# Orbiter-Finance/Plonky2-lib

Hardware: AMD Instinct MI355X
Metric: proofs/sec for secp256k1 ECDSA-verify circuit; Goldilocks NTT GB/s vs HBM peak (higher is better)
Workload: dtype u64 (Goldilocks, 64-bit modular integer)

## Files before the change

### include/glp.h

```cpp
#ifndef GLP_H
#define GLP_H
#include <stddef.h>
#include <stdint.h>

#ifdef __cplusplus
extern "C" {
#endif

#if defined(__GNUC__)
#define GLP_API __attribute__((visibility("default")))
#else
#define GLP_API
#endif

#define GLP_OK 0
#define GLP_ERR_ARG (-1)
#define GLP_ERR_HIP (-2)
#define GLP_ERR_UNSUPPORTED (-3)
#define GLP_ERR_NOGPU (-4)
#define GLP_ERR_PROVE (-5)

#define GLP_HASH_POSEIDON 0
#define GLP_HASH_KECCAK25 1

typedef struct glp_ctx glp_ctx;
typedef struct glp_batch glp_batch;

GLP_API const char *glp_last_error(void);
GLP_API const char *glp_version(void);
GLP_API int glp_device_count(void);

GLP_API int glp_ctx_create(int device_id, glp_ctx **out);
GLP_API void glp_ctx_destroy(glp_ctx *ctx);
GLP_API int glp_ctx_synchronize(glp_ctx *ctx);
GLP_API void *glp_ctx_stream(glp_ctx *ctx);
GLP_API int glp_ctx_set_salt_seed(glp_ctx *ctx, const uint64_t seed[4]);

GLP_API int glp_dev_alloc(glp_ctx *ctx, size_t bytes, void **dev_out);
GLP_API int glp_dev_free(glp_ctx *ctx, void *dev);
GLP_API int glp_dev_upload(glp_ctx *ctx, void *dev_dst, const void *host_src, size_t bytes);
GLP_API int glp_dev_download(glp_ctx *ctx, void *host_dst, const void *dev_src, size_t bytes);

GLP_API int glp_ctx_set_profiling(glp_ctx *ctx, int on);
GLP_API int glp_ctx_stage_reset(glp_ctx *ctx);
GLP_API int glp_ctx_stage_count(glp_ctx *ctx);
GLP_API int glp_ctx_stage_get(glp_ctx *ctx, int index, const char **name, float *ms, double *algorithmic_bytes);

GLP_API int glp_poseidon_permute(glp_ctx *ctx, uint64_t *states, size_t count);
GLP_API int glp_fft(glp_ctx *ctx, uint64_t *cols, uint32_t ncols, uint32_t log_n);
GLP_API int glp_ifft(glp_ctx *ctx, uint64_t *cols, uint32_t ncols, uint32_t log_n);
GLP_API int glp_lde(glp_ctx *ctx, const uint64_t *coeffs, uint32_t ncols, uint32_t log_n, uint32_t rate_bits,
            uint64_t shift, uint64_t *out);

GLP_API int glp_fill_random_device(glp_ctx *ctx, uint64_t *dev_out, size_t count, uint64_t seed);

GLP_API int glp_batch_from_values(glp_ctx *ctx, const uint64_t *values, uint32_t ncols, uint32_t log_n,
                          uint32_t rate_bits, uint32_t cap_height, glp_batch **out);
GLP_API int glp_batch_from_values_device(glp_ctx *ctx, const uint64_t *dev_values, uint32_t ncols, uint32_t log_n,
                                 uint32_t rate_bits, uint32_t cap_height, glp_batch **out);
GLP_API int glp_batch_from_coeffs(glp_ctx *ctx, const uint64_t *coeffs, uint32_t ncols, uint32_t log_n,
                          uint32_t rate_bits, uint32_t cap_height, glp_batch **out);
GLP_API int glp_batch_from_coeffs_device(glp_ctx *ctx, const uint64_t *dev_coeffs, uint32_t ncols, uint32_t log_n,
                                 uint32_t rate_bits, uint32_t cap_height, glp_batch **out);
GLP_API int glp_batch_from_values_h(glp_ctx *ctx, const uint64_t *values, uint32_t ncols, uint32_t log_n, uint32_t rate_bits,
                                    uint32_t cap_height, uint32_t hasher, glp_batch **out);
#define GLP_SALT_SIZE 4
#define GLP_SALT_TAG_WIRES 0
#define GLP_SALT_TAG_ZS 1
#define GLP_SALT_TAG_QUOTIENT 2
#define GLP_SALT_TAG_BATCH 3
GLP_API int glp_batch_from_values_salted(glp_ctx *ctx, const uint64_t *values, uint32_t ncols, uint32_t log_n, uint32_t rate_bits,
                                         uint32_t cap_height, uint32_t hasher, const uint64_t seed[4], glp_batch **out);
GLP_API uint32_t glp_batch_leaf_len(const glp_batch *b);
GLP_API int glp_batch_from_coeffs_h(glp_ctx *ctx, const uint64_t *coeffs, uint32_t ncols, uint32_t log_n, uint32_t rate_bits,
                                    uint32_t cap_height, uint32_t hasher, glp_batch **out);
GLP_API int glp_keccak256(glp_ctx *ctx, const uint8_t *msgs, size_t count, size_t len, uint8_t *digests_out);
GLP_API void glp_batch_free(glp_batch *b);
GLP_API int glp_batch_info(const glp_batch *b, uint32_t *ncols, uint32_t *log_n, uint32_t *rate_bits, uint32_t *cap_height);
GLP_API int glp_batch_cap(const glp_batch *b, uint64_t *cap_out);
GLP_API int glp_batch_coeffs(const glp_batch *b, uint32_t col_begin, uint32_t ncols, uint64_t *out);
GLP_API int glp_batch_leaf(const glp_batch *b, uint64_t leaf_index, uint64_t *out );
// ... 184 lines not shown
```

### plonky2-lib_amd/binding.py

```python
import ctypes as C
import os
import re
import subprocess
import weakref

import numpy as np

P = 0xFFFFFFFF00000001
_HERE = os.path.dirname(os.path.abspath(__file__))
_ROOT = os.path.dirname(_HERE)
_SO = os.path.join(_HERE, "libglprover.so")
_lib = None


class GlpError(RuntimeError):
    def __init__(self, code, msg):
        super().__init__("glp error %d: %s" % (code, msg))
        self.code = code


class _Gate(C.Structure):
    _fields_ = [(f, C.c_uint32) for f in ("type", "selector_index", "group_start", "group_end", "row",
                                          "num_constraints", "p0", "p1")]

# ... 32 lines not shown
        args.append("-B")
    subprocess.check_call(args, stdout=subprocess.DEVNULL)
    return _SO


def exported_symbols():
    hdr = open(os.path.join(_ROOT, "include", "glp.h")).read()
    return re.findall(r"GLP_API [^;(]*?(glp_\w+)\(", hdr)


def load_library():
    global _lib
    if _lib is not None:
        return _lib
    if not os.path.exists(_SO):
        raise GlpError(-4, "libglprover.so is not built (run __graft_entry__.build()); there is no CPU fallback")
    L = C.CDLL(_SO)
    vp, u32, u64, sz = C.c_void_p, C.c_uint32, C.c_uint64, C.c_size_t
    L.glp_last_error.restype = C.c_char_p
    L.glp_version.restype = C.c_char_p
    L.glp_ctx_stream.restype = vp
    L.glp_ctx_stream.argtypes = [vp]
    L.glp_batch_num_digests.restype = sz
    L.glp_batch_num_digests.argtypes = [vp]
    sigs = {
        "glp_ctx_create": [C.c_int, C.POINTER(vp)],
        "glp_ctx_destroy": [vp],
        "glp_ctx_synchronize": [vp],
        "glp_ctx_set_profiling": [vp, C.c_int],
        "glp_ctx_stage_reset": [vp],
        "glp_ctx_stage_count": [vp],
        "glp_ctx_stage_get": [vp, C.c_int, C.POINTER(C.c_char_p), C.POINTER(C.c_float), C.POINTER(C.c_double)],
        "glp_poseidon_permute": [vp, vp, sz],
        "glp_fill_random_device": [vp, vp, sz, u64],
        "glp_fft": [vp, vp, u32, u32],
        "glp_ifft": [vp, vp, u32, u32],
        "glp_lde": [vp, vp, u32, u32, u32, u64, vp],
        "glp_batch_from_values": [vp, vp, u32, u32, u32, u32, C.POINTER(vp)],
        "glp_batch_from_values_device": [vp, vp, u32, u32, u32, u32, C.POINTER(vp)],
        "glp_batch_from_coeffs": [vp, vp, u32, u32, u32, u32, C.POINTER(vp)],
        "glp_batch_from_coeffs_device": [vp, vp, u32, u32, u32, u32, C.POINTER(vp)],
        "glp_batch_from_values_h": [vp, vp, u32, u32, u32, u32, u32, C.POINTER(vp)],
        "glp_batch_from_coeffs_h": [vp, vp, u32, u32, u32, u32, u32, C.POINTER(vp)],
        "glp_keccak256": [vp, vp, sz, sz, vp],
        "glp_batch_free": [vp],
        "glp_batch_info": [vp, C.POINTER(u32), C.POINTER(u32), C.POINTER(u32), C.POINTER(u32)],
        "glp_batch_cap": [vp, vp],
        "glp_batch_coeffs": [vp, u32, u32, vp],
        "glp_batch_leaf": [vp, u64, vp],
        "glp_batch_merkle_proof": [vp, u64, vp],
        "glp_batch_digests": [vp, vp],
        "glp_batch_from_values_salted": [vp, vp, u32, u32, u32, u32, u32, vp, C.POINTER(vp)],
        "glp_ctx_set_salt_seed": [vp, vp],
    }
    L.glp_batch_leaf_len.restype = u32
    L.glp_batch_leaf_len.argtypes = [vp]
    for name in ("glp_batch_num_proofs", "glp_fri_num_proofs"):
        getattr(L, name).restype = u32
        getattr(L, name).argtypes = [vp]
    L.glp_proof_words.restype = sz
    L.glp_proof_words.argtypes = [vp]
    L.glp_proof_bytes_len.restype = sz
    L.glp_proof_bytes_len.argtypes = [vp]
    sigs.update({
        "glp_circuit_create": [vp, C.POINTER(_CircuitDesc), C.POINTER(vp)],
        "glp_circuit_create_ex": [vp, C.POINTER(_CircuitDesc), u32, C.POINTER(vp)],
# ... 943 lines not shown
```

### plonky2-lib_amd/csrc/fri_kernels.inc

```
struct ZTArgs { u64 *zt; ext2 zp2[24]; u32 lg; const u64 *zeta_b; size_t zeta_stride; };
template <bool BATCH>
__global__ __launch_bounds__(256) void k_zeta_table(ZTArgs a) {
    const size_t n = (size_t)1 << a.lg;
    const size_t p = (size_t)blockIdx.x * 256 + threadIdx.x;
    if (p >= n) return;
    const u32 k = bitrev32((u32)p, a.lg);
    ext2 acc = e_from(1);
    if constexpr (BATCH) {
        const u64 *z = a.zeta_b + (size_t)blockIdx.y * a.zeta_stride;
        ext2 sq = e_make(z[0], z[1]);
        for (u32 b = 0; b < a.lg; b++) { if ((k >> b) & 1) acc = e_mul(acc, sq); sq = e_sqr(sq); }
        a.zt += (size_t)blockIdx.y * 2 * n;
    } else {
        for (u32 b = 0; b < a.lg; b++) if ((k >> b) & 1) acc = e_mul(acc, a.zp2[b]);
    }
    a.zt[2 * p] = acc.a; a.zt[2 * p + 1] = acc.b;
}
constexpr int OPEN_BLOCKS = 32;
inline u32 open_blocks(size_t n) { return (u32)std::max<size_t>(1, std::min<size_t>(OPEN_BLOCKS, n / 256)); }
__global__ __launch_bounds__(256) void k_open_dot(const u64 *coeffs, const u64 *zt, u64 *partial, u32 lg, size_t coeffs_bstride,
                                                  size_t zt_bstride, size_t partial_bstride) {
    __shared__ u64 sa[256], sb[256];
    coeffs += (size_t)blockIdx.z * coeffs_bstride; zt += (size_t)blockIdx.z * zt_bstride; partial += (size_t)blockIdx.z * partial_bstride;
    const size_t n = (size_t)1 << lg;
// ... 316 lines not shown
    }
    sa[t] = red.a; sb[t] = red.b;
    __syncthreads();
    for (int s = 128; s > 0; s >>= 1) { if ((int)t < s) { sa[t] = add(sa[t], sa[t + s]); sb[t] = add(sb[t], sb[t + s]); } __syncthreads(); }
    if (t == 0) {
        u64 *pp = a.pp + pk * FCM_PP_WORDS;
        const ext2 shift = e_pow(alpha, len);
        pp[2 * b] = sa[0]; pp[2 * b + 1] = sb[0];
        pp[2 * (NP + b)] = a.z[2 * (pk * npoints + b)]; pp[2 * (NP + b) + 1] = a.z[2 * (pk * npoints + b) + 1];
        pp[2 * (2 * NP + b)] = shift.a; pp[2 * (2 * NP + b) + 1] = shift.b;
    }
}
__global__ __launch_bounds__(256) void k_scale_bitrev_pow(u64 *data, u64 base, u32 lg) {
    const size_t n = (size_t)1 << lg;
    const size_t p = (size_t)blockIdx.x * 256 + threadIdx.x;
    if (p >= n) return;
    const u64 f = dpow(base, bitrev32((u32)p, lg));
    data[(size_t)blockIdx.y * n + p] = mul(data[(size_t)blockIdx.y * n + p], f);
}

__global__ __launch_bounds__(256, 4) void k_fri_leaf_hash(const u64 *vals, u64 *digests, u32 lgL, u32 rb, u32 ab, size_t vals_bstride,
                                                       size_t dig_bstride) {
    vals += (size_t)blockIdx.y * vals_bstride; digests += (size_t)blockIdx.y * dig_bstride;
    const size_t L = (size_t)1 << lgL, ncur = L >> rb, nleaves = L >> ab;
    const size_t Mp = (size_t)blockIdx.x * 256 + threadIdx.x;
    if (Mp >= nleaves) return;
    const size_t m = bitrev32((u32)Mp, lgL - ab);
    const u32 arity = 1u << ab;
    u64 s[12];
#pragma unroll
    for (int i = 0; i < 12; i++) s[i] = 0;
    const u64 *re = vals, *im = vals + L;
    u32 fill = 0;
    for (u32 t = 0; t < arity; t++) {
        const size_t i = (size_t)bitrev32(t, ab) * nleaves + Mp;
        const size_t pos = (i & (((size_t)1 << rb) - 1)) * ncur + (i >> rb);
        s[fill++] = re[pos];
        s[fill++] = im[pos];
        if (fill == 8) { if (2 * arity > 4) pos::permute(s); fill = 0; }
    }
    if (fill && 2 * arity > 4) pos::permute(s);
    ulonglong2 d0, d1;
    d0.x = s[0]; d0.y = s[1]; d1.x = s[2]; d1.y = s[3];
    reinterpret_cast<ulonglong2 *>(digests + 4 * m)[0] = d0;
    reinterpret_cast<ulonglong2 *>(digests + 4 * m)[1] = d1;
}
__global__ __launch_bounds__(256) void k_fri_leaf_hash_coop(const u64 *vals, u64 *digests, u32 lgL, u32 rb, u32 ab, size_t vals_bstride,
                                                            size_t dig_bstride) {
    vals += (size_t)blockIdx.y * vals_bstride; digests += (size_t)blockIdx.y * dig_bstride;
    const size_t L = (size_t)1 << lgL, ncur = L >> rb, nleaves = L >> ab;
    const int tid = threadIdx.x, l = tid & 15, lane = tid & 63, group_base = lane & ~15;
    const size_t Mp0 = (size_t)blockIdx.x * 16 + (tid >> 4);
    const bool live = Mp0 < nleaves;
    const size_t Mp = live ? Mp0 : 0;
    const size_t m = bitrev32((u32)Mp, lgL - ab);
    const u32 len = 2u << ab;
    u64 x = 0;
    for (u32 c = 0; c < len; c += 8) {
        if (l < 8 && c + l < len) {
            const u32 e = c + l, t = e >> 1;
            const size_t i = (size_t)bitrev32(t, ab) * nleaves + Mp;
            const size_t pos = (i & (((size_t)1 << rb) - 1)) * ncur + (i >> rb);
            x = vals[(e & 1 ? L : 0) + pos];
        }
        if (len > 4) x = pos::permute_coop(x, l, group_base);
    }
    if (live && l < 4) digests[4 * m + l] = x;
}
__global__ __launch_bounds__(256) void k_fri_leaf_hash_quad(const u64 *vals, u64 *digests, u32 lgL, u32 rb, u32 ab, size_t vals_bstride,
                                                            size_t dig_bstride) {
    vals += (size_t)blockIdx.y * vals_bstride; digests += (size_t)blockIdx.y * dig_bstride;
    const size_t L = (size_t)1 << lgL, ncur = L >> rb, nleaves = L >> ab;
    const int tid = threadIdx.x, q = tid & 3;
    const size_t Mp0 = (size_t)blockIdx.x * 64 + (tid >> 2);
// ... 185 lines not shown
```

### plonky2-lib_amd/csrc/merkle.hip

```cpp
#include "merkle.h"
#include "keccak.h"
#include "poseidon.h"

namespace glp {
using namespace glf;

constexpr size_t MERKLE_COOP_MAX_PARENTS = 8192;

size_t merkle_num_digests(size_t nleaves, int cap_height) {
    size_t t = 0, w = nleaves, cap = (size_t)1 << cap_height;
    for (;;) { t += w; if (w <= cap) break; w >>= 1; }
    return t;
}
size_t merkle_cap_offset(size_t nleaves, int cap_height) {
    return merkle_num_digests(nleaves, cap_height) - ((size_t)1 << cap_height);
}

__device__ __forceinline__ void store_digest(u64 *dst, const u64 s[12]) {
    ulonglong2 a, b;
    a.x = s[0]; a.y = s[1]; b.x = s[2]; b.y = s[3];
    reinterpret_cast<ulonglong2 *>(dst)[0] = a;
    reinterpret_cast<ulonglong2 *>(dst)[1] = b;
}

__global__ __launch_bounds__(256, 4) void k_leaf_hash_lde(const u64 *__restrict__ lde, u64 *__restrict__ digests,
                                                       u32 ncols, int lg, int rate_bits, size_t lde_stride, size_t dig_stride) {
    lde += (size_t)blockIdx.y * lde_stride; digests += (size_t)blockIdx.y * dig_stride;
    const size_t N = (size_t)1 << (lg + rate_bits);
    const size_t pos = (size_t)blockIdx.x * 256 + threadIdx.x;
    if (pos >= N) return;
    const u32 r = (u32)(pos >> lg), q = (u32)(pos & (((size_t)1 << lg) - 1));
    const size_t leaf = ((size_t)bitrev32(r, rate_bits) << lg) | bitrev32(q, lg);
    u64 s[12];
#pragma unroll
    for (int i = 0; i < 12; i++) s[i] = 0;
    const u64 *p = lde + pos;
    if (ncols <= 4) {
        for (u32 c = 0; c < ncols; c++) s[c] = p[(size_t)c * N];
    } else {
        u64 nx[8];
#pragma unroll
        for (int i = 0; i < 8; i++) nx[i] = i < (int)ncols ? p[(size_t)i * N] : 0;
        for (u32 c = 0; c < ncols; c += 8) {
#pragma unroll
            for (int i = 0; i < 8; i++)
                if (c + i < ncols) s[i] = nx[i];
            if (c + 8 < ncols) {
#pragma unroll
                for (int i = 0; i < 8; i++)
                    if (c + 8 + i < ncols) nx[i] = p[(size_t)(c + 8 + i) * N];
            }
            pos::permute(s);
        }
    }
    store_digest(digests + 4 * leaf, s);
}

__global__ __launch_bounds__(256) void k_leaf_hash_lde_coop(const u64 *__restrict__ lde, u64 *__restrict__ digests,
                                                            u32 ncols, int lg, int rate_bits, size_t lde_stride, size_t dig_stride) {
    lde += (size_t)blockIdx.y * lde_stride; digests += (size_t)blockIdx.y * dig_stride;
    const size_t N = (size_t)1 << (lg + rate_bits);
    const int tid = threadIdx.x, l = tid & 15, lane = tid & 63, group_base = lane & ~15;
    const size_t pos = (size_t)blockIdx.x * 16 + (tid >> 4);
    const bool live = pos < N;
    const size_t p = live ? pos : 0;
    const u32 r = (u32)(p >> lg), q = (u32)(p & (((size_t)1 << lg) - 1));
    const size_t leaf = ((size_t)bitrev32(r, rate_bits) << lg) | bitrev32(q, lg);
    u64 x = 0;
    if (ncols <= 4) {
        if (live && l < 4) digests[4 * leaf + l] = (u32)l < ncols ? lde[(size_t)l * N + p] : 0;
        return;
    }
    for (u32 c = 0; c < ncols; c += 8) {
        if (l < 8 && c + l < ncols) x = lde[(size_t)(c + l) * N + p];
        x = pos::permute_coop(x, l, group_base);
    }
    if (live && l < 4) digests[4 * leaf + l] = x;
}

__global__ __launch_bounds__(256) void k_leaf_hash_lde_quad(const u64 *__restrict__ lde, u64 *__restrict__ digests,
                                                            u32 ncols, int lg, int rate_bits, size_t lde_stride, size_t dig_stride) {
    lde += (size_t)blockIdx.y * lde_stride; digests += (size_t)blockIdx.y * dig_stride;
    const size_t N = (size_t)1 << (lg + rate_bits);
    const int tid = threadIdx.x, q = tid & 3;
    const size_t pos = (size_t)blockIdx.x * 64 + (tid >> 2);
// ... 5 lines not shown
        if (live) digests[4 * leaf + q] = (u32)q < ncols ? lde[(size_t)q * N + p] : 0;
        return;
    }
    u64 x[3] = {0, 0, 0};
    for (u32 c = 0; c < ncols; c += 8) {
#pragma unroll
        for (int s = 0; s < 3; s++) {
            const u32 e = 3 * q + s;
            if (e < 8 && c + e < ncols) x[s] = lde[(size_t)(c + e) * N + p];
        }
        pos::permute_quad(x, q);
    }
    if (live) {
        if (q == 0) { digests[4 * leaf] = x[0]; digests[4 * leaf + 1] = x[1]; digests[4 * leaf + 2] = x[2]; }
        if (q == 1) digests[4 * leaf + 3] = x[0];
    }
}

__global__ __launch_bounds__(256, 4) void k_leaf_hash_rows(const u64 *__restrict__ rows, u64 *__restrict__ digests,
                                                        size_t nleaves, u32 leaf_len) {
    const size_t j = (size_t)blockIdx.x * 256 + threadIdx.x;
    if (j >= nleaves) return;
    u64 s[12];
#pragma unroll
    for (int i = 0; i < 12; i++) s[i] = 0;
    const u64 *p = rows + j * leaf_len;
    if (leaf_len <= 4) {
        for (u32 c = 0; c < leaf_len; c++) s[c] = p[c];
    } else {
        u32 c = 0;
        for (; c + 8 <= leaf_len; c += 8) {
#pragma unroll
            for (int i = 0; i < 8; i++) s[i] = p[c + i];
            pos::permute(s);
        }
        if (c < leaf_len) {
#pragma unroll
            for (int i = 0; i < 8; i++)
                if (c + i < leaf_len) s[i] = p[c + i];
            pos::permute(s);
        }
    }
    store_digest(digests + 4 * j, s);
}

__global__ __launch_bounds__(256) void k_merkle_level(const u64 *__restrict__ in, u64 *__restrict__ out, size_t m, size_t dig_stride) {
    in += (size_t)blockIdx.y * dig_stride; out += (size_t)blockIdx.y * dig_stride;
    const size_t i = (size_t)blockIdx.x * 256 + threadIdx.x;
    if (i >= m) return;
    const ulonglong2 *src = reinterpret_cast<const ulonglong2 *>(in + 8 * i);
    ulonglong2 a = src[0], b = src[1], c2 = src[2], d = src[3];
    u64 s[12] = {a.x, a.y, b.x, b.y, c2.x, c2.y, d.x, d.y, 0, 0, 0, 0};
    pos::permute(s);
    store_digest(out + 4 * i, s);
}

__global__ __launch_bounds__(256) void k_merkle_level_coop(const u64 *__restrict__ in, u64 *__restrict__ out, size_t m, size_t dig_stride) {
    in += (size_t)blockIdx.y * dig_stride; out += (size_t)blockIdx.y * dig_stride;
    const int tid = threadIdx.x, l = tid & 15, lane = tid & 63, group_base = lane & ~15;
    const size_t i = (size_t)blockIdx.x * 16 + (tid >> 4);
    const bool live = i < m;
    u64 x = (live && l < 8) ? in[8 * i + l] : 0;
    x = pos::permute_coop(x, l, group_base);
    if (live && l < 4) out[4 * i + l] = x;
}

__global__ __launch_bounds__(256) void k_merkle_level_quad(const u64 *__restrict__ in, u64 *__restrict__ out, size_t m, size_t dig_stride) {
    in += (size_t)blockIdx.y * dig_stride; out += (size_t)blockIdx.y * dig_stride;
    const int tid = threadIdx.x, q = tid & 3;
    const size_t i0 = (size_t)blockIdx.x * 64 + (tid >> 2);
    const bool live = i0 < m;
    const size_t i = live ? i0 : 0;
    u64 x[3];
#pragma unroll
    for (int s = 0; s < 3; s++) x[s] = 3 * q + s < 8 ? in[8 * i + 3 * q + s] : 0;
    pos::permute_quad(x, q);
    if (live) {
        if (q == 0) { out[4 * i] = x[0]; out[4 * i + 1] = x[1]; out[4 * i + 2] = x[2]; }
        if (q == 1) out[4 * i + 3] = x[0];
    }
}

__global__ void k_permute_states(u64 *states, size_t count) {
    const size_t i = (size_t)blockIdx.x * blockDim.x + threadIdx.x;
    if (i >= count) return;
    u64 s[12];
#pragma unroll
    for (int k = 0; k < 12; k++) s[k] = states[12 * i + k];
    pos::permute(s);
#pragma unroll
    for (int k = 0; k < 12; k++) states[12 * i + k] = s[k];
}

__global__ __launch_bounds__(256) void k_leaf_hash_lde_keccak(const u64 *__restrict__ lde, u64 *__restrict__ digests, u32 ncols, int lg,
                                                              int rate_bits, size_t lde_stride, size_t dig_stride) {
    lde += (size_t)blockIdx.y * lde_stride; digests += (size_t)blockIdx.y * dig_stride;
    const size_t N = (size_t)1 << (lg + rate_bits);
    const size_t pos = (size_t)blockIdx.x * 256 + threadIdx.x;
    if (pos >= N) return;
    const u32 r = (u32)(pos >> lg), q = (u32)(pos & (((size_t)1 << lg) - 1));
    const size_t leaf = ((size_t)bitrev32(r, rate_bits) << lg) | bitrev32(q, lg);
    const u64 *p = lde + pos;
    u64 d[4] = {0, 0, 0, 0};
    if (ncols <= 3) {
        for (u32 c = 0; c < ncols; c++) d[c] = p[(size_t)c * N];
    } else {
        kec::Sponge s;
        kec::sponge_init(s);
        u32 c = 0;
        for (; c + kec::RATE_LANES <= ncols; c += kec::RATE_LANES) {
#pragma unroll
            for (int i = 0; i < kec::RATE_LANES; i++) s.a[i] ^= p[(size_t)(c + i) * N];
            kec::f1600(s.a);
        }
#pragma unroll
        for (int i = 0; i < kec::RATE_LANES; i++) if (c + i < ncols) s.a[i] ^= p[(size_t)(c + i) * N];
        s.fill = (int)(ncols - c);
        kec::sponge_finish(s);
        kec::sponge_digest25(s, d);
    }
    store_digest(digests + 4 * leaf, d);
}
__global__ __launch_bounds__(256) void k_merkle_level_keccak(const u64 *__restrict__ in, u64 *__restrict__ out, size_t m, size_t dig_stride) {
    in += (size_t)blockIdx.y * dig_stride; out += (size_t)blockIdx.y * dig_stride;
    const size_t i = (size_t)blockIdx.x * 256 + threadIdx.x;
    if (i >= m) return;
    const ulonglong2 *src = reinterpret_cast<const ulonglong2 *>(in + 8 * i);
    const ulonglong2 a = src[0], b = src[1], c2 = src[2], e = src[3];
    const u64 l[4] = {a.x, a.y, b.x, b.y}, r[4] = {c2.x, c2.y, e.x, e.y};
    u64 d[4];
    kec::two_to_one(l, r, d);
    store_digest(out + 4 * i, d);
}

static int build_levels(glp_ctx *c, u64 *dev_digests, size_t nleaves, int cap_height, u32 K = 1, size_t dig_stride = 0, int hasher = 0) {
    size_t w = nleaves, cap = (size_t)1 << cap_height;
    u64 *lvl = dev_digests;
    while (w > cap) {
        u64 *nxt = lvl + 4 * w;
        size_t m = w >> 1;
        if (hasher == GLP_HASH_KECCAK25)
            hipLaunchKernelGGL(k_merkle_level_keccak, dim3((unsigned)((m + 255) / 256), K), dim3(256), 0, c->stream, lvl, nxt, m, dig_stride);
        else if (m * K <= MERKLE_COOP_MAX_PARENTS)
            hipLaunchKernelGGL(k_merkle_level_coop, dim3((unsigned)((m + 15) / 16), K), dim3(256), 0, c->stream, lvl, nxt, m, dig_stride);
        else if (m * K <= c->merkle_quad_max)
            hipLaunchKernelGGL(k_merkle_level_quad, dim3((unsigned)((m + 63) / 64), K), dim3(256), 0, c->stream, lvl, nxt, m, dig_stride);
        else
            hipLaunchKernelGGL(k_merkle_level, dim3((unsigned)((m + 255) / 256), K), dim3(256), 0, c->stream, lvl, nxt, m, dig_stride);
        GLP_HIP(hipGetLastError());
        lvl = nxt; w = m;
    }
    return GLP_OK;
}

int merkle_levels(glp_ctx *c, u64 *dev_digests, size_t nleaves, int cap_height, u32 K, size_t dig_stride, int hasher) {
    return build_levels(c, dev_digests, nleaves, cap_height, K, dig_stride, hasher);
}

int merkle_from_lde(glp_ctx *c, const u64 *dev_lde, u32 ncols, int lg, int rate_bits, int cap_height, u64 *dev_digests, u32 K,
                    size_t lde_stride, size_t dig_stride, int hasher) {
    const size_t N = (size_t)1 << (lg + rate_bits);
    if (cap_height < 0 || ((size_t)1 << cap_height) > N)
        return set_error(GLP_ERR_ARG, "cap_height=%d should be at most log2(leaves)=%d", cap_height, lg + rate_bits);
    GLP_REQUIRE(K >= 1 && K <= 65535, "batch of %u trees outside 1..65535", K);
    {
        StageScope st(c, "merkle_leaves", (double)N * K * (8.0 * ncols + 32.0));
        if (hasher == GLP_HASH_KECCAK25)
            hipLaunchKernelGGL(k_leaf_hash_lde_keccak, dim3((unsigned)((N + 255) / 256), K), dim3(256), 0, c->stream, dev_lde, dev_digests,
                               ncols, lg, rate_bits, lde_stride, dig_stride);
        else if (N * K <= c->merkle_coop_max)
            hipLaunchKernelGGL(k_leaf_hash_lde_coop, dim3((unsigned)((N + 15) / 16), K), dim3(256), 0, c->stream, dev_lde, dev_digests,
                               ncols, lg, rate_bits, lde_stride, dig_stride);
        else if (N * K <= c->merkle_quad_max)
// ... 72 lines not shown
__global__ __launch_bounds__(256) void k_salt_lde(u64 *__restrict__ lde, u32 ncols, int lg, int rate_bits, size_t lde_stride,
                                                  u64 seed0, u64 seed1, u64 seed2, u64 seed3, u32 tag) {
    lde += (size_t)blockIdx.y * lde_stride;
    const size_t N = (size_t)1 << (lg + rate_bits);
    const size_t pos = (size_t)blockIdx.x * 256 + threadIdx.x;
    if (pos >= N) return;
    const u32 r = (u32)(pos >> lg), q = (u32)(pos & (((size_t)1 << lg) - 1));
    const u64 leaf = ((u64)bitrev32(r, rate_bits) << lg) | bitrev32(q, lg);
    u64 s[12] = {seed0, seed1, seed2, add(seed3, (u64)blockIdx.y), (u64)tag, leaf & 0xffffffffull, leaf >> 32, 0, 0, 0, 0, 0};
    pos::permute(s);
#pragma unroll
    for (int i = 0; i < 4; i++) lde[(size_t)(ncols + i) * N + pos] = s[i];
}

int merkle_fill_salts(glp_ctx *c, u64 *dev_lde, u32 ncols, int lg, int rate_bits, const u64 seed[4], u32 tag, u32 K, size_t lde_stride) {
    const size_t N = (size_t)1 << (lg + rate_bits);
    GLP_REQUIRE(K >= 1 && K <= 65535, "batch of %u trees outside 1..65535", K);
    for (int i = 0; i < 4; i++) GLP_REQUIRE(seed[i] < P, "salt seed word %d is not a canonical field element", i);
    StageScope st(c, "salt", (double)N * K * 32.0);
    hipLaunchKernelGGL(k_salt_lde, dim3((unsigned)((N + 255) / 256), K), dim3(256), 0, c->stream, dev_lde, ncols, lg, rate_bits, lde_stride,
                       seed[0], seed[1], seed[2], seed[3], tag);
    GLP_HIP(hipGetLastError());
    return GLP_OK;
}

int poseidon_permute_states(glp_ctx *c, u64 *dev_states, size_t count) {
    if (!count) return GLP_OK;
    hipLaunchKernelGGL(k_permute_states, dim3((unsigned)((count + 255) / 256)), dim3(256), 0, c->stream, dev_states, count);
    GLP_HIP(hipGetLastError());
    return GLP_OK;
}

}
```

### plonky2-lib_amd/csrc/poseidon.h

```cpp
#pragma once
#include "glf.h"
#include "poseidon_rc.inc"

namespace pos {
using namespace glf;

#if defined(__HIP_DEVICE_COMPILE__)
static __device__ const u64 RC[360] = { GLP_POSEIDON_RC_LIST };
#else
static const u64 RC[360] = { GLP_POSEIDON_RC_LIST };
#endif

GLF_HD u64 sbox7(u64 x) {
    u64 x2 = sqr(x), x4 = sqr(x2), x3 = mul(x, x2);
    return mul(x3, x4);
}

GLF_HD void mds_layer(u64 s[12]) {
    constexpr u32 C[12] = {17, 15, 41, 16, 2, 28, 13, 13, 39, 18, 34, 20};
    u32 lo[12], hi[12];
#pragma unroll
    for (int i = 0; i < 12; i++) { lo[i] = (u32)s[i]; hi[i] = (u32)(s[i] >> 32); }
#pragma unroll
    for (int r = 0; r < 12; r++) {
// ... 75 lines not shown
        for (int r = 0; r < 12; r++) {
            u64 acc = 0;
            for (int k = 1; k < 12; k++) acc += m_at(r, k) * t.bt[s - 1][k];
            t.bt[s][r] = (u32)acc;
        }
    for (int r = 0; r < 12; r++) {
        u64 w = 0;
        for (int c = 0; c < 12; c++) { w += G[r][c]; if (G[r][c] >> 32) w = ~0ULL >> 1; }
        for (int i = 1; i <= K; i++) w += t.bt[K - i][r];
        if (w > t.max_weight) t.max_weight = w;
    }
    return t;
}
template <int K> struct BlkConst { u64 kpre; u64 k0[K]; u64 kK[12]; };
template <int K, bool MERGED> constexpr BlkConst<K> make_blk(int first_round) {
    BlkConst<K> b{};
    u64 kc[12] = {}, nx[12] = {};
    for (int i = 0; i < 12; i++) kc[i] = RC_CE[12 * (first_round + (MERGED ? 0 : 1)) + i];
    b.kpre = MERGED ? kc[0] : 0;
    for (int j = MERGED ? 1 : 2; j <= K; j++) {
        for (int r = 0; r < 12; r++) {
            unsigned __int128 acc = RC_CE[12 * (first_round + j) + r];
            for (int k = 1; k < 12; k++) acc += (unsigned __int128)m_at(r, k) * kc[k];
            nx[r] = (u64)(acc % PRIME);
        }
        for (int r = 0; r < 12; r++) kc[r] = nx[r];
        if (j < K) b.k0[j - 1] = kc[0];
    }
    if (!MERGED && K > 1) b.k0[0] = RC_CE[12 * (first_round + 1)];
    b.k0[K - 1] = 0;
    for (int r = 0; r < 12; r++) b.kK[r] = kc[r];
    return b;
}
}

#if defined(__HIP_DEVICE_COMPILE__)
static __device__ const u64 RC_ZERO[12] = {0, 0, 0, 0, 0, 0, 0, 0, 0, 0, 0, 0};

__device__ __forceinline__ u64 sbox7_nc(u64 x) {
#ifdef GLP_SBOX_PLAIN_MUL
    const u64 x2 = mul_nc(x, x), x4 = mul_nc(x2, x2), x3 = mul_nc(x, x2);
    return mul_nc(x3, x4);
#else
    const u64 x2 = mul_nc_cc(x, x), x4 = mul_nc_cc(x2, x2), x3 = mul_nc_cc(x, x2);
    return mul_nc_cc(x3, x4);
#endif
}
#ifndef GLP_MDS_GROUP
#define GLP_MDS_GROUP 4
#endif
#ifndef GLP_SBOX_GROUP
#define GLP_SBOX_GROUP 4
#endif
__device__ __forceinline__ void sbox_layer_nc(u64 s[12]) {
#pragma unroll
    for (int i = 0; i < 12; i++) {
        s[i] = sbox7_nc(s[i]);
        if (i % GLP_SBOX_GROUP == GLP_SBOX_GROUP - 1) __builtin_amdgcn_sched_barrier(0);
    }
}
__device__ __forceinline__ void mds_add_nc(u64 s[12], const u64 *rc) {
    constexpr u32 C[12] = {17, 15, 41, 16, 2, 28, 13, 13, 39, 18, 34, 20};
    u32 lo[12], hi[12];
#pragma unroll
    for (int i = 0; i < 12; i++) { lo[i] = (u32)s[i]; hi[i] = (u32)(s[i] >> 32); }
    u32 c16 = 16, c2 = 2;
    asm volatile("" : "+s"(c16), "+s"(c2));
#pragma unroll
    for (int r = 0; r < 12; r++) {
        u64 al = (u64)(u32)rc[r] + (u64)lo[r] * (r == 0 ? C[0] + 8 : C[0]);
        asm("" : "+v"(al));
#pragma unroll
        for (int i = 1; i < 12; i++) al += (u64)lo[(i + r) % 12] * (C[i] == 16 ? c16 : C[i] == 2 ? c2 : C[i]);
        u64 ah = (al >> 32) + (rc[r] >> 32);
#pragma unroll
        for (int i = 0; i < 12; i++) ah += (u64)hi[(i + r) % 12] * (i == 0 && r == 0 ? C[0] + 8 : C[i] == 16 ? c16 : C[i] == 2 ? c2 : C[i]);
#ifdef GLP_MDS_FOLD_C
        s[r] = fold96_c((ah << 32) | (u32)al, (u32)(ah >> 32));
#else
        s[r] = fold96_nc((ah << 32) | (u32)al, (u32)(ah >> 32));
#endif
        if (r % GLP_MDS_GROUP == GLP_MDS_GROUP - 1) __builtin_amdgcn_sched_barrier(0);
    }
}

static __device__ const pblk::BlkConst<3> PBM[1] = {pblk::make_blk<3, true>(4)};
static __device__ const pblk::BlkConst<4> PB4[4] = {pblk::make_blk<4, false>(7), pblk::make_blk<4, false>(11),
                                                    pblk::make_blk<4, false>(15), pblk::make_blk<4, false>(19)};
static __device__ const pblk::BlkConst<3> PB3[1] = {pblk::make_blk<3, false>(23)};

#define GLP_PB_ROW(OUT, GROW, KCONST, NS, BCOEF)                                                    \
    do {                                                                                            \
        const u64 _k = (KCONST);                                                                    \
        u64 al = (u32)_k;                                                                           \
        _Pragma("unroll") for (int c = 0; c < 12; c++) if ((GROW)[c] != 0) al += (u64)lo[c] * (GROW)[c];   \
        _Pragma("unroll") for (int i = 0; i < (NS); i++) al += (u64)slo[i] * (BCOEF);               \
        u64 ah = (al >> 32) + (_k >> 32);                                                           \
        _Pragma("unroll") for (int c = 0; c < 12; c++) if ((GROW)[c] != 0) ah += (u64)hi[c] * (GROW)[c];   \
        _Pragma("unroll") for (int i = 0; i < (NS); i++) ah += (u64)shi[i] * (BCOEF);               \
        (OUT) = fold96_nc((ah << 32) | (u32)al, (u32)(ah >> 32));                                   \
    } while (0)

template <int K, bool MERGED, class Hook>
__device__ __forceinline__ void partial_block_nc(u64 s[12], const pblk::BlkConst<K> &kc, Hook hook) {
    constexpr pblk::Tab<K, MERGED> T = pblk::make_tab<K, MERGED>();
    static_assert(T.max_weight + 2 < (1ULL << 32), "unreduced accumulation would overflow");
    u32 lo[12], hi[12], slo[K], shi[K];
#pragma unroll
    for (int i = 0; i < 12; i++) { lo[i] = (u32)s[i]; hi[i] = (u32)(s[i] >> 32); }
    u64 x0 = s[0];
    if constexpr (MERGED) {
        constexpr u32 MROW0[12] = {25, 15, 41, 16, 2, 28, 13, 13, 39, 18, 34, 20};
        GLP_PB_ROW(x0, MROW0, kc.kpre, 0, 0u);
    }
    u64 sig = sbox7_nc(hook(0, x0));
    slo[0] = (u32)sig; shi[0] = (u32)(sig >> 32);
#pragma unroll
    for (int j = 1; j < K; j++) {
        u64 z;
        GLP_PB_ROW(z, T.g0[j - 1], kc.k0[j - 1], j, T.bt[j - 1 - i][0]);
        sig = sbox7_nc(hook(j, z));
        slo[j] = (u32)sig; shi[j] = (u32)(sig >> 32);
    }
#pragma unroll
    for (int r = 0; r < 12; r++) {
        GLP_PB_ROW(s[r], T.gK[r], kc.kK[r], K, T.bt[K - 1 - i][r]);
        if (r % GLP_MDS_GROUP == GLP_MDS_GROUP - 1) __builtin_amdgcn_sched_barrier(0);
    }
}

template <int K, bool MERGED>
__device__ __forceinline__ void partial_block_nc(u64 s[12], const pblk::BlkConst<K> &kc) {
    partial_block_nc<K, MERGED>(s, kc, [](int, u64 z) { return z; });
}

struct FullNext { u64 k[8][12]; };
constexpr FullNext make_full_next() {
    FullNext f{};
    for (int r = 0; r < 3; r++) for (int i = 0; i < 12; i++) { f.k[r][i] = pblk::RC_CE[12 * (r + 1) + i]; f.k[4 + r][i] = pblk::RC_CE[12 * (27 + r) + i]; }
    return f;
}
static __device__ const FullNext RCN = make_full_next();

__device__ __forceinline__ void permute(u64 s[12]) {
#pragma unroll
    for (int i = 0; i < 12; i++) s[i] = add(s[i], RC[i]);
#ifdef GLP_POSEIDON_PLAIN_PARTIAL
    int rc = 12;
    for (int r = 0; r < 4; r++) { sbox_layer_nc(s); mds_add_nc(s, RC + rc); rc += 12; }
    for (int r = 0; r < 22; r++) { s[0] = sbox7_nc(s[0]); mds_add_nc(s, RC + rc); rc += 12; }
    for (int r = 0; r < 3; r++) { sbox_layer_nc(s); mds_add_nc(s, RC + rc); rc += 12; }
    sbox_layer_nc(s);
    mds_add_nc(s, RC_ZERO);
#else
#ifdef GLP_POSEIDON_FLAT
#define GLP_FULL_ROUND(i) sbox_layer_nc(s); mds_add_nc(s, RCN.k[i]);
    GLP_FULL_ROUND(0) GLP_FULL_ROUND(1) GLP_FULL_ROUND(2)
    sbox_layer_nc(s);
    partial_block_nc<3, true>(s, PBM[0]);
    partial_block_nc<4, false>(s, PB4[0]); partial_block_nc<4, false>(s, PB4[1]);
    partial_block_nc<4, false>(s, PB4[2]); partial_block_nc<4, false>(s, PB4[3]);
    partial_block_nc<3, false>(s, PB3[0]);
    GLP_FULL_ROUND(4) GLP_FULL_ROUND(5) GLP_FULL_ROUND(6) GLP_FULL_ROUND(7)
#undef GLP_FULL_ROUND
#else
#pragma nounroll
    for (int half = 0; half < 2; half++) {
#pragma nounroll
        for (int r = 0; r < 4; r++) {
            sbox_layer_nc(s);
            if (half == 0 && r == 3) break;
            mds_add_nc(s, RCN.k[4 * half + r]);
        }
        if (half == 0) {
            partial_block_nc<3, true>(s, PBM[0]);
#pragma nounroll
            for (int b = 0; b < 4; b++) partial_block_nc<4, false>(s, PB4[b]);
            partial_block_nc<3, false>(s, PB3[0]);
        }
    }
#endif
#endif
#pragma unroll
    for (int i = 0; i < 12; i++) s[i] = canon(s[i]);
}
__device__ __forceinline__ void pow_round0_consts(const u64 st[12], u32 pos, u64 out[12]) {
    u64 c[12];
    for (int i = 0; i < 12; i++) c[i] = (u32)i == pos ? 0 : canon(sbox7_nc(add(st[i], RC[i])));
    for (int r = 0; r < 12; r++) {
        u64 acc = RC[12 + r];
        for (int i = 0; i < 12; i++) if ((u32)i != pos) acc = add(acc, mul(c[i], (u64)mds_entry(r, i)));
        out[r] = acc;
    }
}
template <class GiveUp>
__device__ __forceinline__ u64 permute_tail7(u64 s[12], GiveUp give_up) {
#pragma nounroll
    for (int half = 0; half < 2; half++) {
#pragma nounroll
        for (int r = half == 0 ? 1 : 0; r < 4; r++) {
            sbox_layer_nc(s);
            if (r == 3) break;
            mds_add_nc(s, RCN.k[4 * half + r]);
            if (half == 1 && r == 1 && give_up()) return ~0ull;
        }
        if (half == 0) {
            if (give_up()) return ~0ull;
            partial_block_nc<3, true>(s, PBM[0]);
#pragma nounroll
            for (int b = 0; b < 4; b++) {
                partial_block_nc<4, false>(s, PB4[b]);
                if (b == 1 && give_up()) return ~0ull;
            }
            partial_block_nc<3, false>(s, PB3[0]);
            if (give_up()) return ~0ull;
// ... 105 lines not shown
template <int K, bool MERGED>
inline void partial_block(u64 s[12], const pblk::BlkConst<K> &kc) {
    constexpr pblk::Tab<K, MERGED> T = pblk::make_tab<K, MERGED>();
    static_assert(T.max_weight + 2 < (1ULL << 32), "unreduced accumulation would overflow");
    u32 lo[12], hi[12], slo[K], shi[K];
    for (int i = 0; i < 12; i++) { lo[i] = (u32)s[i]; hi[i] = (u32)(s[i] >> 32); }
    u64 x0 = s[0];
    if (MERGED) {
        constexpr u32 MROW0[12] = {25, 15, 41, 16, 2, 28, 13, 13, 39, 18, 34, 20};
        u64 al = 0, ah = 0;
        _Pragma("unroll") for (int c = 0; c < 12; c++) { al += (u64)lo[c] * MROW0[c]; ah += (u64)hi[c] * MROW0[c]; }
        x0 = fold(al, ah, kc.kpre);
    }
    u64 sig = sbox(x0);
    slo[0] = (u32)sig; shi[0] = (u32)(sig >> 32);
    _Pragma("unroll") for (int j = 1; j < K; j++) {
        u64 al = 0, ah = 0;
        _Pragma("unroll") for (int c = 0; c < 12; c++) { al += (u64)lo[c] * T.g0[j - 1][c]; ah += (u64)hi[c] * T.g0[j - 1][c]; }
        _Pragma("unroll") for (int i = 0; i < j; i++) { al += (u64)slo[i] * T.bt[j - 1 - i][0]; ah += (u64)shi[i] * T.bt[j - 1 - i][0]; }
        sig = sbox(fold(al, ah, kc.k0[j - 1]));
        slo[j] = (u32)sig; shi[j] = (u32)(sig >> 32);
    }
    _Pragma("unroll") for (int r = 0; r < 12; r++) {
        u64 al = 0, ah = 0;
        _Pragma("unroll") for (int c = 0; c < 12; c++) { al += (u64)lo[c] * T.gK[r][c]; ah += (u64)hi[c] * T.gK[r][c]; }
        _Pragma("unroll") for (int i = 0; i < K; i++) { al += (u64)slo[i] * T.bt[K - 1 - i][r]; ah += (u64)shi[i] * T.bt[K - 1 - i][r]; }
        s[r] = fold(al, ah, kc.kK[r]);
    }
}
static constexpr pblk::BlkConst<3> HPBM = pblk::make_blk<3, true>(4);
static constexpr pblk::BlkConst<4> HPB4[4] = {pblk::make_blk<4, false>(7), pblk::make_blk<4, false>(11), pblk::make_blk<4, false>(15), pblk::make_blk<4, false>(19)};
static constexpr pblk::BlkConst<3> HPB3 = pblk::make_blk<3, false>(23);
}
inline void permute(u64 s[12]) {
    static const u64 ZERO12[12] = {0, 0, 0, 0, 0, 0, 0, 0, 0, 0, 0, 0};
    for (int i = 0; i < 12; i++) s[i] = add(s[i], RC[i]);
    for (int r = 0; r < 4; r++) {
        for (int i = 0; i < 12; i++) s[i] = host::sbox(s[i]);
        if (r < 3) host::mds_add(s, RC + 12 * (r + 1));
    }
    host::partial_block<3, true>(s, host::HPBM);
    for (int b = 0; b < 4; b++) host::partial_block<4, false>(s, host::HPB4[b]);
    host::partial_block<3, false>(s, host::HPB3);
    for (int r = 26; r < 30; r++) {
        for (int i = 0; i < 12; i++) s[i] = host::sbox(s[i]);
        host::mds_add(s, r < 29 ? RC + 12 * (r + 1) : ZERO12);
    }
    for (int i = 0; i < 12; i++) s[i] = canon(canon(s[i]));
}
inline u64 permute_coop(u64 x, int, int) { return x; }
inline void permute_quad(u64 *, int) {}
GLF_HD u64 sbox7_nc(u64 x) { return x; }
GLF_HD void pow_round0_consts(const u64 *, u32, u64 *) {}
GLF_HD u64 permute_tail7(u64 *) { return 0; }
template <class GiveUp> GLF_HD u64 permute_tail7(u64 *, GiveUp) { return 0; }
GLF_HD u64 shfl64(u64 v, int) { return v; }
GLF_HD u64 shfl_xor64(u64 v, int) { return v; }
#endif

GLF_HD void two_to_one(const u64 l[4], const u64 r[4], u64 out[4]) {
    u64 s[12];
#pragma unroll
    for (int i = 0; i < 4; i++) { s[i] = l[i]; s[4 + i] = r[i]; s[8 + i] = 0; }
    permute(s);
#pragma unroll
    for (int i = 0; i < 4; i++) out[i] = s[i];
}
// ... 3 lines not shown
```

### profiles/isa_slots.py

```python
#!/usr/bin/env python3
import collections
import json
import os
import re
import subprocess
import sys
import tempfile

ROOT = os.path.dirname(os.path.dirname(os.path.abspath(__file__)))
HALF_WEIGHT = 1.75
FULL = {"v_add_u32_e32", "v_sub_u32_e32", "v_subrev_u32_e32", "v_xor_b32_e32", "v_and_b32_e32", "v_or_b32_e32", "v_mov_b32_e32",
        "v_lshrrev_b32_e32", "v_not_b32_e32", "v_cndmask_b32_e32", "v_accvgpr_write_b32", "v_accvgpr_read_b32"}


def main():
    src = os.path.join(ROOT, "plonky2-lib_amd", "csrc", "merkle.hip")
    with tempfile.TemporaryDirectory() as td:
        out = os.path.join(td, "merkle.s")
        subprocess.check_call(["/opt/rocm/bin/hipcc", "--offload-arch=gfx950", "-O3", "-std=c++17", "-DGLP_LDE_NO_HOIST", "-DGLP_POSEIDON_FLAT", "-S", "--cuda-device-only",
                               "-o", out, src], stderr=subprocess.DEVNULL)
        txt = open(out).read()
    body = txt[txt.index("_ZN3glp16k_permute_statesEPmm:"):]
    body = body[:body.index("s_endpgm")]
    ops = []
    labels = set()
    for l in body.split("\n"):
        m = re.match(r"^(\.LBB\d+_\d+):", l)
        if m:
            labels.add(m.group(1))
            continue
        m = re.match(r"^\s+([vs]_\w+|ds_\w+|global_\w+)(.*)", l)
        if m:
            if m.group(1).startswith("s_cbranch") and any(lab in m.group(2) for lab in labels):
                raise SystemExit("backward branch in the flat build: loops were not fully unrolled")
            ops.append(m.group(1))
    c = collections.Counter(ops)
    valu = sum(v for k, v in c.items() if k.startswith("v_"))
    slots = sum(v * (1.0 if k in FULL else HALF_WEIGHT) for k, v in c.items() if k.startswith("v_"))
    out = {"build": "-DGLP_POSEIDON_FLAT (all round loops unrolled; the shipped build keeps them rolled: same instructions per round)",
           "mads_per_permutation": c["v_mad_u64_u32"], "valu_instructions": valu, "s_nop": c["s_nop"],
           "full_rate_instructions": sum(v for k, v in c.items() if k in FULL),
           "slots_per_permutation": slots, "top_opcodes": dict(c.most_common(14))}
    json.dump(out, sys.stdout, indent=1)
    print()


if __name__ == "__main__":
    main()
```

Before: 9.080.

## Specialize Poseidon for zero-capacity entry and digest-only exit, add fused Merkle tail kernel

Adds flags to the device Poseidon permutation. On the first absorption, when the capacity lanes are zero, it skips their round-constant add and S-box and folds the first MDS contribution of the capacity into precomputed constants. On the last absorption it computes only the four digest outputs of the final MDS. It also adds a k_merkle_tail kernel that hashes the last Merkle levels for the non-Keccak hasher in one launch, keeping intermediate nodes in shared memory. This saves arithmetic in leaf and node hashing and avoids per-level launches, at the cost of more code paths and branch-dependent specialization in the rolled loop.

Result: no change. 9.134 (median of 6 runs) (+0.6%).

```diff
diff --git a/include/glp.h b/include/glp.h
--- a/include/glp.h
+++ b/include/glp.h
@@ -47,6 +47,7 @@
 GLP_API int glp_ctx_stage_get(glp_ctx *ctx, int index, const char **name, float *ms, double *algorithmic_bytes);
 
 GLP_API int glp_poseidon_permute(glp_ctx *ctx, uint64_t *states, size_t count);
+GLP_API int glp_poseidon_zero_cap_entry(uint64_t out[16]);
 GLP_API int glp_fft(glp_ctx *ctx, uint64_t *cols, uint32_t ncols, uint32_t log_n);
 GLP_API int glp_ifft(glp_ctx *ctx, uint64_t *cols, uint32_t ncols, uint32_t log_n);
 GLP_API int glp_lde(glp_ctx *ctx, const uint64_t *coeffs, uint32_t ncols, uint32_t log_n, uint32_t rate_bits,
diff --git a/plonky2-lib_amd/binding.py b/plonky2-lib_amd/binding.py
--- a/plonky2-lib_amd/binding.py
+++ b/plonky2-lib_amd/binding.py
@@ -88,6 +88,7 @@
         "glp_ctx_stage_count": [vp],
         "glp_ctx_stage_get": [vp, C.c_int, C.POINTER(C.c_char_p), C.POINTER(C.c_float), C.POINTER(C.c_double)],
         "glp_poseidon_permute": [vp, vp, sz],
+        "glp_poseidon_zero_cap_entry": [vp],
         "glp_fill_random_device": [vp, vp, sz, u64],
         "glp_fft": [vp, vp, u32, u32],
         "glp_ifft": [vp, vp, u32, u32],
diff --git a/plonky2-lib_amd/csrc/fri_kernels.inc b/plonky2-lib_amd/csrc/fri_kernels.inc
--- a/plonky2-lib_amd/csrc/fri_kernels.inc
+++ b/plonky2-lib_amd/csrc/fri_kernels.inc
@@ -372,14 +372,15 @@
     for (int i = 0; i < 12; i++) s[i] = 0;
     const u64 *re = vals, *im = vals + L;
     u32 fill = 0;
+    bool first = true;
     for (u32 t = 0; t < arity; t++) {
         const size_t i = (size_t)bitrev32(t, ab) * nleaves + Mp;
         const size_t pos = (i & (((size_t)1 << rb) - 1)) * ncur + (i >> rb);
         s[fill++] = re[pos];
         s[fill++] = im[pos];
-        if (fill == 8) { if (2 * arity > 4) pos::permute(s); fill = 0; }
-    }
-    if (fill && 2 * arity > 4) pos::permute(s);
+        if (fill == 8) { if (2 * arity > 4) pos::permute(s, first, t + 1 == arity); fill = 0; first = false; }
+    }
+    if (fill && 2 * arity > 4) pos::permute(s, first, true);
     ulonglong2 d0, d1;
     d0.x = s[0]; d0.y = s[1]; d1.x = s[2]; d1.y = s[3];
     reinterpret_cast<ulonglong2 *>(digests + 4 * m)[0] = d0;
diff --git a/plonky2-lib_amd/csrc/merkle.hip b/plonky2-lib_amd/csrc/merkle.hip
--- a/plonky2-lib_amd/csrc/merkle.hip
+++ b/plonky2-lib_amd/csrc/merkle.hip
@@ -50,7 +50,7 @@
                 for (int i = 0; i < 8; i++)
                     if (c + 8 + i < ncols) nx[i] = p[(size_t)(c + 8 + i) * N];
             }
-            pos::permute(s);
+            pos::permute(s, c == 0, c + 8 >= ncols);
         }
     }
     store_digest(digests + 4 * leaf, s);
@@ -122,13 +122,13 @@
         for (; c + 8 <= leaf_len; c += 8) {
 #pragma unroll
             for (int i = 0; i < 8; i++) s[i] = p[c + i];
-            pos::permute(s);
+            pos::permute(s, c == 0, c + 8 >= leaf_len);
         }
         if (c < leaf_len) {
 #pragma unroll
             for (int i = 0; i < 8; i++)
                 if (c + i < leaf_len) s[i] = p[c + i];
-            pos::permute(s);
+            pos::permute(s, c == 0, true);
         }
     }
     store_digest(digests + 4 * j, s);
@@ -141,7 +141,7 @@
     const ulonglong2 *src = reinterpret_cast<const ulonglong2 *>(in + 8 * i);
     ulonglong2 a = src[0], b = src[1], c2 = src[2], d = src[3];
     u64 s[12] = {a.x, a.y, b.x, b.y, c2.x, c2.y, d.x, d.y, 0, 0, 0, 0};
-    pos::permute(s);
+    pos::permute(s, true, true);
     store_digest(out + 4 * i, s);
 }
 
@@ -168,6 +168,51 @@
     if (live) {
         if (q == 0) { out[4 * i] = x[0]; out[4 * i + 1] = x[1]; out[4 * i + 2] = x[2]; }
         if (q == 1) out[4 * i + 3] = x[0];
+    }
+}
+
+#ifndef GLP_MERKLE_TAIL_NODES
+#define GLP_MERKLE_TAIL_NODES 128
+#endif
+constexpr u32 MERKLE_TAIL_NODES = GLP_MERKLE_TAIL_NODES;
+__global__ __launch_bounds__(256) void k_merkle_tail(u64 *__restrict__ dig, size_t off, size_t w, u32 lg_n0, u32 nlevels, size_t dig_stride) {
+    __shared__ u64 lv[2][MERKLE_TAIL_NODES * 4];
+    dig += (size_t)blockIdx.y * dig_stride;
+    const u32 tid = threadIdx.x, n0 = 1u << lg_n0;
+    for (u32 i = tid; i < 4 * n0; i += 256) lv[0][i] = dig[4 * (off + (size_t)blockIdx.x * n0) + i];
+    __syncthreads();
+    u32 n = n0;
+    for (u32 lev = 0; lev < nlevels; lev++) {
+        const u64 *cur = lv[lev & 1];
+        u64 *nxt = lv[(lev & 1) ^ 1];
+        const u32 m = n >> 1;
+        off += w; w >>= 1;
+        u64 *out = dig + 4 * (off + (size_t)blockIdx.x * m);
+        if (m > 16) {
+            const int q = tid & 3;
+            for (u32 base = 0; base < m; base += 64) {
+                const u32 i = base + (tid >> 2);
+                const bool live = i < m;
+                if (base + 16 * (tid >> 6) >= m) break;
+                u64 x[3];
+#pragma unroll
+                for (int s = 0; s < 3; s++) x[s] = live && 3 * q + s < 8 ? cur[8 * i + 3 * q + s] : 0;
+                pos::permute_quad(x, q);
+                if (live) {
+                    if (q == 0) { nxt[4 * i] = x[0]; nxt[4 * i + 1] = x[1]; nxt[4 * i + 2] = x[2]; out[4 * i] = x[0]; out[4 * i + 1] = x[1]; out[4 * i + 2] = x[2]; }
+                    if (q == 1) { nxt[4 * i + 3] = x[0]; out[4 * i + 3] = x[0]; }
+                }
+            }
+        } else if (4 * (tid >> 6) < m) {
+            const int l = tid & 15;
+            const u32 i = tid >> 4;
+            const bool live = i < m;
+            u64 x = live && l < 8 ? cur[8 * i + l] : 0;
+            x = pos::permute_coop(x, l, (int)(tid & 48));
+            if (live && l < 4) { nxt[4 * i + l] = x; out[4 * i + l] = x; }
+        }
+        __syncthreads();
+        n = m;
     }
 }
 
@@ -229,6 +274,15 @@
     while (w > cap) {
         u64 *nxt = lvl + 4 * w;
         size_t m = w >> 1;
+        if (hasher != GLP_HASH_KECCAK25 && (w >> cap_height) <= MERKLE_TAIL_NODES) {
+            u32 lg_n0 = 0, nlevels = 0;
+            while (((size_t)2 << lg_n0) <= w && (2u << lg_n0) <= MERKLE_TAIL_NODES) lg_n0++;
+            while ((w >> nlevels) > cap) nlevels++;
+            hipLaunchKernelGGL(k_merkle_tail, dim3((unsigned)(w >> lg_n0), K), dim3(256), 0, c->stream, dev_digests, (size_t)((lvl - dev_digests) / 4), w,
+                               lg_n0, nlevels, dig_stride);
+            GLP_HIP(hipGetLastError());
+            break;
+        }
         if (hasher == GLP_HASH_KECCAK25)
             hipLaunchKernelGGL(k_merkle_level_keccak, dim3((unsigned)((m + 255) / 256), K), dim3(256), 0, c->stream, lvl, nxt, m, dig_stride);
         else if (m * K <= MERKLE_COOP_MAX_PARENTS)
@@ -367,3 +421,12 @@
 }
 
 }
+
+extern "C" int glp_poseidon_zero_cap_entry(uint64_t out[16]) {
+    using namespace glp;
+    GLP_REQUIRE(out, "null argument");
+    constexpr pos::pblk::ZeroCapEntry z = pos::pblk::make_zero_cap_entry();
+    for (int i = 0; i < 4; i++) out[i] = z.sb[i];
+    for (int r = 0; r < 12; r++) out[4 + r] = z.k[r];
+    return GLP_OK;
+}
diff --git a/plonky2-lib_amd/csrc/poseidon.h b/plonky2-lib_amd/csrc/poseidon.h
--- a/plonky2-lib_amd/csrc/poseidon.h
+++ b/plonky2-lib_amd/csrc/poseidon.h
@@ -131,6 +131,21 @@
     for (int r = 0; r < 12; r++) b.kK[r] = kc[r];
     return b;
 }
+struct ZeroCapEntry { u64 sb[4]; u64 k[12]; };
+constexpr u64 ce_mul(u64 a, u64 b) { return (u64)((unsigned __int128)a * b % PRIME); }
+constexpr ZeroCapEntry make_zero_cap_entry() {
+    ZeroCapEntry z{};
+    for (int i = 0; i < 4; i++) {
+        const u64 x = RC_CE[8 + i] % PRIME, x2 = ce_mul(x, x), x4 = ce_mul(x2, x2), x3 = ce_mul(x, x2);
+        z.sb[i] = ce_mul(x3, x4);
+    }
+    for (int r = 0; r < 12; r++) {
+        unsigned __int128 acc = RC_CE[12 + r];
+        for (int i = 0; i < 4; i++) acc += (unsigned __int128)m_at(r, 8 + i) * z.sb[i];
+        z.k[r] = (u64)(acc % PRIME);
+    }
+    return z;
+}
 }
 
 #if defined(__HIP_DEVICE_COMPILE__)
@@ -151,29 +166,37 @@
 #ifndef GLP_SBOX_GROUP
 #define GLP_SBOX_GROUP 4
 #endif
-__device__ __forceinline__ void sbox_layer_nc(u64 s[12]) {
-#pragma unroll
-    for (int i = 0; i < 12; i++) {
+__device__ __forceinline__ void sbox_layer_nc(u64 s[12], bool skip_capacity = false) {
+#pragma unroll
+    for (int i = 0; i < 8; i++) {
         s[i] = sbox7_nc(s[i]);
         if (i % GLP_SBOX_GROUP == GLP_SBOX_GROUP - 1) __builtin_amdgcn_sched_barrier(0);
     }
-}
-__device__ __forceinline__ void mds_add_nc(u64 s[12], const u64 *rc) {
+    if (skip_capacity) return;
+#pragma unroll
+    for (int i = 8; i < 12; i++) {
+        s[i] = sbox7_nc(s[i]);
+        if (i % GLP_SBOX_GROUP == GLP_SBOX_GROUP - 1) __builtin_amdgcn_sched_barrier(0);
+    }
+}
+template <int NIN, int NOUT>
+__device__ __forceinline__ void mds_add_nc_t(u64 s[12], const u64 *rc) {
     constexpr u32 C[12] = {17, 15, 41, 16, 2, 28, 13, 13, 39, 18, 34, 20};
     u32 lo[12], hi[12];
 #pragma unroll
-    for (int i = 0; i < 12; i++) { lo[i] = (u32)s[i]; hi[i] = (u32)(s[i] >> 32); }
+    for (int i = 0; i < NIN; i++) { lo[i] = (u32)s[i]; hi[i] = (u32)(s[i] >> 32); }
     u32 c16 = 16, c2 = 2;
     asm volatile("" : "+s"(c16), "+s"(c2));
 #pragma unroll
-    for (int r = 0; r < 12; r++) {
-        u64 al = (u64)(u32)rc[r] + (u64)lo[r] * (r == 0 ? C[0] + 8 : C[0]);
+    for (int r = 0; r < NOUT; r++) {
+        u64 al = (u64)(u32)rc[r];
+        if (r < NIN) al += (u64)lo[r] * (r == 0 ? C[0] + 8 : C[0]);
         asm("" : "+v"(al));
 #pragma unroll
-        for (int i = 1; i < 12; i++) al += (u64)lo[(i + r) % 12] * (C[i] == 16 ? c16 : C[i] == 2 ? c2 : C[i]);
+        for (int i = 1; i < 12; i++) if ((i + r) % 12 < NIN) al += (u64)lo[(i + r) % 12] * (C[i] == 16 ? c16 : C[i] == 2 ? c2 : C[i]);
         u64 ah = (al >> 32) + (rc[r] >> 32);
 #pragma unroll
-        for (int i = 0; i < 12; i++) ah += (u64)hi[(i + r) % 12] * (i == 0 && r == 0 ? C[0] + 8 : C[i] == 16 ? c16 : C[i] == 2 ? c2 : C[i]);
+        for (int i = 0; i < 12; i++) if ((i + r) % 12 < NIN) ah += (u64)hi[(i + r) % 12] * (i == 0 && r == 0 ? C[0] + 8 : C[i] == 16 ? c16 : C[i] == 2 ? c2 : C[i]);
 #ifdef GLP_MDS_FOLD_C
         s[r] = fold96_c((ah << 32) | (u32)al, (u32)(ah >> 32));
 #else
@@ -182,6 +205,7 @@
         if (r % GLP_MDS_GROUP == GLP_MDS_GROUP - 1) __builtin_amdgcn_sched_barrier(0);
     }
 }
+__device__ __forceinline__ void mds_add_nc(u64 s[12], const u64 *rc) { mds_add_nc_t<12, 12>(s, rc); }
 
 static __device__ const pblk::BlkConst<3> PBM[1] = {pblk::make_blk<3, true>(4)};
 static __device__ const pblk::BlkConst<4> PB4[4] = {pblk::make_blk<4, false>(7), pblk::make_blk<4, false>(11),
@@ -241,9 +265,17 @@
 }
 static __device__ const FullNext RCN = make_full_next();
 
-__device__ __forceinline__ void permute(u64 s[12]) {
-#pragma unroll
-    for (int i = 0; i < 12; i++) s[i] = add(s[i], RC[i]);
+static __device__ const pblk::ZeroCapEntry ZCE = pblk::make_zero_cap_entry();
+__device__ __forceinline__ void permute(u64 s[12], bool zero_cap = false, bool digest_only = false) {
+#ifdef GLP_POSEIDON_PLAIN_PARTIAL
+    zero_cap = digest_only = false;
+#endif
+#pragma unroll
+    for (int i = 0; i < 8; i++) s[i] = add(s[i], RC[i]);
+    if (!zero_cap) {
+#pragma unroll
+        for (int i = 8; i < 12; i++) s[i] = add(s[i], RC[i]);
+    }
 #ifdef GLP_POSEIDON_PLAIN_PARTIAL
     int rc = 12;
     for (int r = 0; r < 4; r++) { sbox_layer_nc(s); mds_add_nc(s, RC + rc); rc += 12; }
@@ -254,22 +286,27 @@
 #else
 #ifdef GLP_POSEIDON_FLAT
 #define GLP_FULL_ROUND(i) sbox_layer_nc(s); mds_add_nc(s, RCN.k[i]);
-    GLP_FULL_ROUND(0) GLP_FULL_ROUND(1) GLP_FULL_ROUND(2)
+    if (zero_cap) { sbox_layer_nc(s, true); mds_add_nc_t<8, 12>(s, ZCE.k); } else { GLP_FULL_ROUND(0) }
+    GLP_FULL_ROUND(1) GLP_FULL_ROUND(2)
     sbox_layer_nc(s);
     partial_block_nc<3, true>(s, PBM[0]);
     partial_block_nc<4, false>(s, PB4[0]); partial_block_nc<4, false>(s, PB4[1]);
     partial_block_nc<4, false>(s, PB4[2]); partial_block_nc<4, false>(s, PB4[3]);
     partial_block_nc<3, false>(s, PB3[0]);
-    GLP_FULL_ROUND(4) GLP_FULL_ROUND(5) GLP_FULL_ROUND(6) GLP_FULL_ROUND(7)
+    GLP_FULL_ROUND(4) GLP_FULL_ROUND(5) GLP_FULL_ROUND(6)
+    sbox_layer_nc(s);
+    if (!digest_only) mds_add_nc(s, RCN.k[7]);
 #undef GLP_FULL_ROUND
 #else
 #pragma nounroll
     for (int half = 0; half < 2; half++) {
 #pragma nounroll
         for (int r = 0; r < 4; r++) {
-            sbox_layer_nc(s);
-            if (half == 0 && r == 3) break;
-            mds_add_nc(s, RCN.k[4 * half + r]);
+            const bool entry = zero_cap && half == 0 && r == 0;
+            sbox_layer_nc(s, entry);
+            if (r == 3 && (half == 0 || digest_only)) break;
+            if (entry) mds_add_nc_t<8, 12>(s, ZCE.k);
+            else mds_add_nc(s, RCN.k[4 * half + r]);
         }
         if (half == 0) {
             partial_block_nc<3, true>(s, PBM[0]);
@@ -280,6 +317,12 @@
     }
 #endif
 #endif
+    if (digest_only) {
+        mds_add_nc_t<12, 4>(s, RCN.k[7]);
+#pragma unroll
+        for (int i = 0; i < 4; i++) s[i] = canon(s[i]);
+        return;
+    }
 #pragma unroll
     for (int i = 0; i < 12; i++) s[i] = canon(s[i]);
 }
@@ -451,7 +494,7 @@
 static constexpr pblk::BlkConst<4> HPB4[4] = {pblk::make_blk<4, false>(7), pblk::make_blk<4, false>(11), pblk::make_blk<4, false>(15), pblk::make_blk<4, false>(19)};
 static constexpr pblk::BlkConst<3> HPB3 = pblk::make_blk<3, false>(23);
 }
-inline void permute(u64 s[12]) {
+inline void permute(u64 s[12], bool = false, bool = false) {
     static const u64 ZERO12[12] = {0, 0, 0, 0, 0, 0, 0, 0, 0, 0, 0, 0};
     for (int i = 0; i < 12; i++) s[i] = add(s[i], RC[i]);
     for (int r = 0; r < 4; r++) {
diff --git a/profiles/isa_slots.py b/profiles/isa_slots.py
--- a/profiles/isa_slots.py
+++ b/profiles/isa_slots.py
@@ -20,7 +20,8 @@
         subprocess.check_call(["/opt/rocm/bin/hipcc", "--offload-arch=gfx950", "-O3", "-std=c++17", "-DGLP_LDE_NO_HOIST", "-DGLP_POSEIDON_FLAT", "-S", "--cuda-device-only",
                                "-o", out, src], stderr=subprocess.DEVNULL)
         txt = open(out).read()
-    body = txt[txt.index("_ZN3glp16k_permute_statesEPmm:"):]
+    kernel = sys.argv[1] if len(sys.argv) > 1 else "_ZN3glp16k_permute_statesEPmm"
+    body = txt[txt.index(kernel + ":"):]
     body = body[:body.index("s_endpgm")]
     ops = []
     labels = set()
@@ -37,7 +38,7 @@
     c = collections.Counter(ops)
     valu = sum(v for k, v in c.items() if k.startswith("v_"))
     slots = sum(v * (1.0 if k in FULL else HALF_WEIGHT) for k, v in c.items() if k.startswith("v_"))
-    out = {"build": "-DGLP_POSEIDON_FLAT (all round loops unrolled; the shipped build keeps them rolled: same instructions per round)",
+    out = {"kernel": kernel, "build": "-DGLP_POSEIDON_FLAT (all round loops unrolled; the shipped build keeps them rolled: same instructions per round)",
            "mads_per_permutation": c["v_mad_u64_u32"], "valu_instructions": valu, "s_nop": c["s_nop"],
            "full_rate_instructions": sum(v for k, v in c.items() if k in FULL),
            "slots_per_permutation": slots, "top_opcodes": dict(c.most_common(14))}
```
